# emstoudenmire/TNML

Measured on AMD Instinct MI355X. Metric: two-site bond updates/sec, higher is better.
Workload: dtype f64; 1 GPU; fixedL N=784, maxm=120, 60000 images (BASELINE config 3: its 60 000 images on 1 GPU instead of 8), Npass=4, lambda=0.001, minm=120, fp64 throughout; random-init W at m=maxm; timed bonds 405..202 (consecutive interior bonds, Label-carrying shiftE on each, m=119); global_images=60000, sites=784, maxm=120, parallelism=dp1 (image sharding + RCCL all-reduce), rccl_ranks=1

## Files before the change

### tnml_amd/csrc/kernels_grad.hip

```cpp
#include "tnml_internal.h"

typedef double f64x4g __attribute__((ext_vector_type(4)));

#define GQ_TI 32
#ifndef GQ_SLOT
#define GQ_SLOT(rgp) (2 * (rgp))
#endif
#ifndef GQ_PRIO
#define GQ_PRIO 3
#endif
#define GQ_RS 34
#define GQ_Q 32
#define GQ_E_D_N(NR) (32 * (NR) * GQ_RS)
#define GQ_Z_D (GQ_Q * GQ_RS)
#define GQ_W_D (4 * GQ_RS)
#define GQ_LDS_DOUBLES_N(NR) (2 * (GQ_E_D_N(NR) + GQ_Z_D + GQ_W_D))
#define GQ_LDS_DOUBLES GQ_LDS_DOUBLES_N(4)

struct GradQuadArgs {
    const double* EI; const double* phiI; const double* phiO;
    const double* EL; size_t EL_lstride;
    const double* dP;
    int NTp;
    int mI, mO, Kp, Np;
    double* slab;
    int ngroups, per, nchunks;
    long long* dbg = nullptr;
};

static __device__ __forceinline__ void gq_barrier() {
    asm volatile("s_waitcnt lgkmcnt(0)" ::: "memory");
    __builtin_amdgcn_s_barrier();
    asm volatile("" ::: "memory");
}

template <int ABL, int NR = 4>
__global__ __launch_bounds__(1024) void k_grad_quad(GradQuadArgs A) {
    static_assert(NR == 4 || NR == 2, "quad form or pair form");
    constexpr int GQ_E_D = GQ_E_D_N(NR);
    extern __shared__ __attribute__((aligned(16))) double gq_lds[];
    double* const Es = gq_lds;
    double* const Zs = Es + 2 * GQ_E_D;
    double* const Ws = Zs + 2 * GQ_Z_D;
    const int tid = threadIdx.x, lane = tid & 63, w = __builtin_amdgcn_readfirstlane(tid >> 6);
    const int b = blockIdx.x;
    const long long ts0 = (ABL == 5 || ABL == 6) ? (long long)wall_clock64() : 0;
    const int h = (b >> 3) & (NR - 1), grp = (b & 7) + 8 * (NR == 4 ? b >> 5 : b >> 4);
    if (grp >= A.ngroups) return;
    const int NTp = A.NTp;
    const int c0 = grp * A.per;
    const int nch = min(A.per, A.nchunks - c0);
    auto n_of = [&](int k) { return (size_t)(c0 + (k < nch ? k : nch - 1)) * GQ_TI; };

    const int rho = lane >> 4, x2 = 2 * (lane & 15);
    double2 pc[3];
    const unsigned pvoff = (unsigned)(((size_t)rho * NTp + x2) * sizeof(double));
    auto ld16 = [&](const double* ubase, unsigned voff) { return *reinterpret_cast<const double2*>(reinterpret_cast<const char*>(ubase) + voff); };
    const bool v0 = 4 * w + rho < A.mI, v1 = NR == 4 && 64 + 4 * w + rho < A.mI;
    const double* fO = A.phiO - 2 * (size_t)NTp;
    const double* fb = A.phiI < fO ? A.phiI : fO;
    const unsigned fvoff = pvoff + (unsigned)(((rho < 2 ? A.phiI : fO) - fb) * (ptrdiff_t)sizeof(double));
    auto piece_load = [&](size_t nE, double2 (&pc)[3]) {
        unsigned vo = pvoff, vf = fvoff;
        asm volatile("" : "+v"(vo), "+v"(vf));
        pc[0] = v0 ? ld16(A.EI + (size_t)(4 * w) * NTp + nE, vo) : make_double2(0., 0.);
        if (NR == 4) pc[1] = v1 ? ld16(A.EI + (size_t)(4 * (w + 16)) * NTp + nE, vo) : make_double2(0., 0.);
        if (w == 15) pc[2] = ld16(fb + nE, vf);
    };
    const int dst0 = (4 * w + rho) * GQ_RS + x2;
    auto piece_store = [&](int bufE, const double2 (&pc)[3]) {
        *reinterpret_cast<double2*>(Es + bufE * GQ_E_D + dst0) = pc[0];
        if (NR == 4) *reinterpret_cast<double2*>(Es + bufE * GQ_E_D + dst0 + 64 * GQ_RS) = pc[1];
        if (w == 15) {
            const int lI = 16 * (rho >> 1) + (lane & 15), lO = 16 * (2 + (rho & 1)) + (lane & 15);
            const double ix = __shfl(pc[2].x, lI), iy = __shfl(pc[2].y, lI), ox = __shfl(pc[2].x, lO), oy = __shfl(pc[2].y, lO);
            *reinterpret_cast<double2*>(Ws + bufE * GQ_W_D + rho * GQ_RS + x2) = make_double2(ix * ox, iy * oy);
        }
    };
    const int img = lane & 31, qs = lane >> 5;
    double el[2][5], dpv[5];
    const unsigned elvoff = (unsigned)(((size_t)(5 * qs) * A.EL_lstride + img) * sizeof(double));
    const unsigned dpvoff = (unsigned)(((size_t)(5 * qs) * NTp + img) * sizeof(double));
    const bool uv[2] = {GQ_Q * h + w < A.mO, GQ_Q * h + w + 16 < A.mO};
    auto el_load = [&](size_t n0, double (&el)[2][5], double (&dpv)[5]) {
        unsigned elvo = elvoff, dpvo = dpvoff;
        asm volatile("" : "+v"(elvo), "+v"(dpvo));
#pragma unroll
        for (int l = 0; l < 5; ++l) dpv[l] = *reinterpret_cast<const double*>(reinterpret_cast<const char*>(A.dP + (size_t)l * NTp + n0) + dpvo);
#pragma unroll
        for (int j = 0; j < 2; ++j) {
            const double* ub = A.EL + (size_t)(GQ_Q * h + w + 16 * j) * NTp + n0;
#pragma unroll
            for (int l = 0; l < 5; ++l)
                el[j][l] = !uv[j] ? 0. : (ABL == 1 ? 1.0 : *reinterpret_cast<const double*>(reinterpret_cast<const char*>(ub + (size_t)l * A.EL_lstride) + elvo));
        }
    };
    auto z_build = [&](int bufZ, const double (&el)[2][5], const double (&dpv)[5]) {
#pragma unroll
        for (int j = 0; j < 2; ++j) {
            double z = 0.;
#pragma unroll
            for (int l = 0; l < 5; ++l) z = fma(el[j][l], dpv[l], z);
            const double zo = __shfl_xor(z, 32);
            if (qs == 0) Zs[bufZ * GQ_Z_D + (w + 16 * j) * GQ_RS + img] = z + zo;
        }
    };

    const int rgp = w >> 2, J = w & 3;
    const int li = lane & 15, g = lane >> 4;
    const int sI = rgp >> 1, a0 = 16 * NR * (rgp & 1);
    const int eoff = (a0 + li) * GQ_RS + g;
    const int cc = 16 * J + li;
    const int zoff = (cc >> 1) * GQ_RS + g;
    const int woff = (2 * sI + (cc & 1)) * GQ_RS + g;
    {
        double2 pc0[3]; double el0[2][5], dpv0[5];
        piece_load(n_of(0), pc0);
        el_load(n_of(0), el0, dpv0);
        if (ABL != 6) { piece_load(n_of(1), pc); el_load(n_of(1), el, dpv); }
        piece_store(0, pc0);
        z_build(0, el0, dpv0);
        if (ABL == 6) { piece_load(n_of(1), pc); el_load(n_of(1), el, dpv); }
    }
    gq_barrier();
    const long long ts1 = (ABL == 5 || ABL == 6) ? (long long)wall_clock64() : 0;

    f64x4g acc[NR];
#pragma unroll
    for (int r = 0; r < NR; ++r) acc[r] = f64x4g{0., 0., 0., 0.};
    double en[NR], zn, on;
    auto frag_load = [&](int buf, int ks) {
        const double* Eb = Es + buf * GQ_E_D + eoff + 4 * ks;
#pragma unroll
        for (int r = 0; r < NR; ++r) en[r] = Eb[16 * r * GQ_RS];
        zn = Zs[buf * GQ_Z_D + zoff + 4 * ks];
        on = Ws[buf * GQ_W_D + woff + 4 * ks];
    };
    frag_load(0, 0);
    for (int k = 0; k < nch; ++k) {
        const int cur = k & 1, nxt = cur ^ 1;
#pragma unroll
        for (int ks = 0; ks < 8; ++ks) {
            if (ABL != 3 && ks == GQ_SLOT(rgp)) {
                __builtin_amdgcn_s_setprio(GQ_PRIO);
                piece_store(nxt, pc);
                z_build(nxt, el, dpv);
                piece_load(n_of(k + 2), pc);
                el_load(n_of(k + 2), el, dpv);
                __builtin_amdgcn_s_setprio(0);
                __builtin_amdgcn_sched_barrier(0);
            }
            double ec[NR];
#pragma unroll
            for (int r = 0; r < NR; ++r) ec[r] = en[r];
            const double bc = zn * on;
            __builtin_amdgcn_sched_barrier(0);
            if (ks < 7) frag_load(cur, ks + 1);
            __builtin_amdgcn_sched_barrier(0);
#pragma unroll
            for (int r = 0; r < NR; ++r) acc[r] = __builtin_amdgcn_mfma_f64_16x16x4f64(ec[r], bc, acc[r], 0, 0, 0);
            __builtin_amdgcn_sched_barrier(0);
        }
        gq_barrier();
        frag_load(nxt, 0);
    }

    const long long ts2 = (ABL == 5 || ABL == 6) ? (long long)wall_clock64() : 0;
    double* out = A.slab + (size_t)grp * A.Kp * A.Np;
    const int col = 2 * GQ_Q * h + cc;
    if (col < A.Np) {
#pragma unroll
        for (int r = 0; r < NR; ++r)
#pragma unroll
            for (int e4 = 0; e4 < 4; ++e4) {
                const int row = 2 * (a0 + 16 * r + g + 4 * e4) + sI;
                if (row < A.Kp) out[(size_t)row * A.Np + col] = acc[r][e4];
            }
    }
    if ((ABL == 5 || ABL == 6) && A.dbg) {
        asm volatile("s_waitcnt vmcnt(0)" ::: "memory");
        __syncthreads();
        if (tid == 0) { long long* d = A.dbg + 4 * (size_t)b; d[0] = ts0; d[1] = ts1; d[2] = ts2; d[3] = (long long)wall_clock64(); }
    }
}

static inline bool gq_pair_form(const Bgemm64Args& a) { return a.mI <= 64 && a.mO <= 64 && a.Kp <= 128 && a.Np <= 128; }

bool grad_quad_applies(const tnml_ctx* c, const Bgemm64Args& a) {
    if (!c->grad_quad || !a.EL || !a.env64 || a.L != 1 || a.w) return false;
    if (a.mI < 1 || a.mO < 1 || a.mI > 128 || a.mO > 128 || a.Kp < 2 * a.mI || a.Np < 2 * a.mO || a.Kp > 256 || a.Np > 256 || a.NTp % GQ_TI) return false;
    if (c->grad_quad == 1) {
        if (gq_pair_form(a)) {
            const int mm = a.mI * a.mO;
            if (!c->grad_pair || a.NTp < 15360 || mm < 33 * 33 || mm > 56 * 56) return false;
        } else if (a.NTp < 4096 || a.mI * a.mO < 72 * 72) return false;
    }
    if ((size_t)TNML_NL * a.EL_lstride * sizeof(double) >= ((size_t)1 << 32)) return false;
    return c->slab_bytes >= (size_t)64 * a.Kp * a.Np * sizeof(double);
}

template <int NR>
static int grad_quad_go(tnml_ctx* c, const GradQuadArgs& K, int grid) {
    const size_t lds = sizeof(double) * GQ_LDS_DOUBLES_N(NR);
    bool& done = NR == 4 ? c->attr_gq : c->attr_gp;
    if (!done) {
        if (hipFuncSetAttribute(reinterpret_cast<const void*>(k_grad_quad<0, NR>), hipFuncAttributeMaxDynamicSharedMemorySize, (int)lds) != hipSuccess)
            return tnml_fail(c, "grad_quad: cannot reserve %zu bytes of LDS", lds);
        done = true;
    }
    ProfScope ps(c, KC_GRAD_QUAD);
    hipLaunchKernelGGL((k_grad_quad<0, NR>), dim3(grid), dim3(1024), lds, c->stream, K);
    return 0;
}

int launch_grad_quad(tnml_ctx* c, const Bgemm64Args& a, double* G) {
    if (!c->cu_count) { hipDeviceProp_t pr; c->cu_count = hipGetDeviceProperties(&pr, c->cfg.device) == hipSuccess ? pr.multiProcessorCount : 256; }
    const bool pair = gq_pair_form(a) && c->grad_pair != 0;
    const int nwg = pair ? 2 : 4;
    GradQuadArgs K;
    K.EI = static_cast<const double*>(a.EI); K.phiI = static_cast<const double*>(a.phiI); K.phiO = static_cast<const double*>(a.phiO);
    K.EL = static_cast<const double*>(a.EL); K.EL_lstride = a.EL_lstride; K.dP = a.dPz; K.NTp = a.NTp;
    K.mI = a.mI; K.mO = a.mO; K.Kp = a.Kp; K.Np = a.Np;
    K.slab = static_cast<double*>(c->slab);
    K.nchunks = a.NTp / GQ_TI;
    int groups = c->cu_count / nwg;
    const int cap = (int)(c->slab_bytes / ((size_t)a.Kp * a.Np * sizeof(double)));
    if (groups > cap) groups = cap;
    if (c->bgemm_wgs > 0 && c->bgemm_wgs / nwg < groups) groups = c->bgemm_wgs / nwg > 0 ? c->bgemm_wgs / nwg : 1;
    if (groups > K.nchunks) groups = K.nchunks;
    K.per = (K.nchunks + groups - 1) / groups;
    K.ngroups = (K.nchunks + K.per - 1) / K.per;
    const int grid = 8 * nwg * ((K.ngroups + 7) / 8);
    if (pair) TCK(grad_quad_go<2>(c, K, grid));
    else      TCK(grad_quad_go<4>(c, K, grid));
    const size_t n = (size_t)a.Kp * a.Np;
    if (c->defer_slab) c->slab_pending = K.ngroups;
    else {
        ProfScope ps(c, KC_SLABRED);
        launch_slab_reduce64(c, static_cast<const double*>(c->slab), G, n, K.ngroups);
    }
    HIPCK(c, hipGetLastError());
    return 0;
}
```

### tnml_amd/csrc/tnml_core.hip

```cpp
#include <algorithm>
#include <climits>
#include <cmath>
#include <cstdarg>
#include <cstdlib>
#include <cstring>

#include "tnml_host.h"

static std::string g_create_err;

int tnml_fail(tnml_ctx* c, const char* fmt, ...) {
    char buf[512];
    va_list ap; va_start(ap, fmt); vsnprintf(buf, sizeof buf, fmt, ap); va_end(ap);
    if (c) { c->err = buf; if (c->local && c->coll_depth > 0) local_comm_abort(c); } else g_create_err = buf;
    return 1;
}
const char* tnml_last_error(const tnml_ctx* c) { return c ? c->err.c_str() : g_create_err.c_str(); }
const char* tnml_last_warning(const tnml_ctx* c) { return c ? c->warn.c_str() : ""; }

static hipEvent_t prof_event(tnml_ctx* c) {
    if (!c->prof_free.empty()) { hipEvent_t e = c->prof_free.back(); c->prof_free.pop_back(); return e; }
    hipEvent_t e; (void)hipEventCreate(&e); return e;
}
void prof_begin(tnml_ctx* c, int, hipEvent_t* e0, hipStream_t st) { *e0 = prof_event(c); (void)hipEventRecord(*e0, st ? st : c->stream); }
void prof_end(tnml_ctx* c, int kc, hipEvent_t e0, hipStream_t st) {
    hipEvent_t e1 = prof_event(c); (void)hipEventRecord(e1, st ? st : c->stream);
    c->prof_pending.push_back({e0, e1, kc});
    if (c->prof_pending.size() > 8192) prof_resolve(c);
}
void prof_resolve(tnml_ctx* c) {
    if (c->prof_pending.empty()) return;
    (void)hipStreamSynchronize(c->stream);
    for (auto& p : c->prof_pending) {
        float ms = 0.f;
        if (hipEventElapsedTime(&ms, p.e0, p.e1) == hipSuccess) { c->prof_ms[p.kc] += ms; c->prof_launches[p.kc] += 1; }
        c->prof_free.push_back(p.e0); c->prof_free.push_back(p.e1);
    }
    c->prof_pending.clear();
}
int tnml_profile_enable(tnml_ctx* c, int on) { prof_resolve(c); c->prof = on != 0; return 0; }
int tnml_profile_select(tnml_ctx* c, const char* class_name) {
    prof_resolve(c);
    if (!class_name || !*class_name) { c->prof_mask = 0xffffffffu; return 0; }
    unsigned mask = 0;
    const char* s = class_name;
    while (*s) {
        const char* e = strchr(s, ',');
        const size_t len = e ? (size_t)(e - s) : strlen(s);
        bool found = false;
        for (int i = 0; i < KC_COUNT; ++i) if (strlen(kclass_names[i]) == len && !strncmp(s, kclass_names[i], len)) { mask |= 1u << i; found = true; }
        if (!found) return tnml_fail(c, "tnml_profile_select: unknown kernel class in %s", class_name);
        s = e ? e + 1 : s + len;
    }
    c->prof_mask = mask;
    return 0;
}
int tnml_profile_count(tnml_ctx*) { return KC_COUNT; }
int tnml_profile_get(tnml_ctx* c, int idx, char* name64, int64_t* launches, double* total_ms) {
    if (idx < 0 || idx >= KC_COUNT) return tnml_fail(c, "profile index out of range");
    prof_resolve(c);
    if (name64) { strncpy(name64, kclass_names[idx], 63); name64[63] = 0; }
    if (launches) *launches = c->prof_launches[idx];
    if (total_ms) *total_ms = c->prof_ms[idx];
    return 0;
}
int tnml_profile_reset(tnml_ctx* c) {
    prof_resolve(c);
    for (int i = 0; i < KC_COUNT; ++i) { c->prof_launches[i] = 0; c->prof_ms[i] = 0.; }
    return 0;
}
enum OptKind { OPT_BOOL, OPT_INT, OPT_REAL };
enum OptHook { HK_NONE, HK_REUSE_P, HK_DEFER_TAIL, HK_CHECK_REPLICAS, HK_ENV_BUDGET, HK_COMM_TIMEOUT, HK_FAIL_SPLIT, HK_MISPREDICT, HK_SVD_PRINT, HK_CG_METHOD, HK_NOISE, HK_PREDICT_TILE };
struct OptDef {
    const char* name; const char* env; OptKind kind;
    int tnml_ctx::* ifield; double tnml_ctx::* rfield;
    double lo, hi; OptHook hook;
};
static const OptDef k_options[] = {
    {"fast_cg",          "TNML_FAST_CG",        OPT_BOOL, &tnml_ctx::fast_cg,             nullptr,          0, 1,       HK_NONE},
    {"reuse_p",          "TNML_REUSE_P",        OPT_BOOL, &tnml_ctx::reuse_p,             nullptr,          0, 1,       HK_REUSE_P},
    {"fuse_z",           "TNML_FUSE_Z",         OPT_BOOL, &tnml_ctx::fuse_z,              nullptr,          0, 1,       HK_NONE},
    {"merged_cg",        "TNML_MERGED_CG",      OPT_INT,  &tnml_ctx::merged_cg,           nullptr,          0, 2,       HK_NONE},
    {"defer_tail",       "TNML_DEFER_TAIL",     OPT_BOOL, &tnml_ctx::defer_tail,          nullptr,          0, 1,       HK_DEFER_TAIL},
    {"check_replicas",   "TNML_CHECK_REPLICAS", OPT_INT,  &tnml_ctx::check_replicas_mode, nullptr,          0, 2,       HK_CHECK_REPLICAS},
    {"fused_fwd",        "TNML_FUSED_FWD",      OPT_INT,  &tnml_ctx::fused_fwd,           nullptr,          0, INT_MAX, HK_NONE},
    {"fwd_res",          "TNML_FWD_RES",        OPT_INT,  &tnml_ctx::fwd_res,             nullptr,          0, 3,       HK_NONE},
    {"shift_res",        "TNML_SHIFT_RES",      OPT_INT,  &tnml_ctx::shift_res,           nullptr,          0, 2,       HK_NONE},
    {"shift_skip",       "TNML_SHIFT_SKIP",     OPT_BOOL, &tnml_ctx::shift_skip,          nullptr,          0, 1,       HK_NONE},
    {"res_grid",         nullptr,               OPT_INT,  &tnml_ctx::res_grid,            nullptr,          0, INT_MAX, HK_NONE},
    {"res_pace",         "TNML_RES_PACE",       OPT_INT,  &tnml_ctx::res_pace,            nullptr,          0, 4,       HK_NONE},
    {"grad_quad",        "TNML_GRAD_QUAD",      OPT_INT,  &tnml_ctx::grad_quad,           nullptr,          0, 2,       HK_NONE},
    {"grad_pair",        "TNML_GRAD_PAIR",      OPT_BOOL, &tnml_ctx::grad_pair,           nullptr,          0, 1,       HK_NONE},
    {"bgemm_wgs",        "TNML_BGEMM_WGS",      OPT_INT,  &tnml_ctx::bgemm_wgs,           nullptr,          0, INT_MAX, HK_NONE},
    {"bgemm_per",        "TNML_BGEMM_PER",      OPT_INT,  &tnml_ctx::bgemm_per,           nullptr,          0, 1 << 20, HK_NONE},
    {"sytrd_exit",       nullptr,               OPT_BOOL, &tnml_ctx::sytrd_exit,          nullptr,          0, 1,       HK_NONE},
    {"bgs_chol",         "TNML_BGS_CHOL",       OPT_BOOL, &tnml_ctx::bgs_chol,            nullptr,          0, 1,       HK_NONE},
    {"spec_split",       "TNML_SPEC_SPLIT",     OPT_BOOL, &tnml_ctx::spec_split,          nullptr,          0, 1,       HK_NONE},
    {"debug_fail_split", nullptr,               OPT_INT,  &tnml_ctx::debug_fail_split,    nullptr,         -1, INT_MAX, HK_FAIL_SPLIT},
    {"spec_predict",     "TNML_SPEC_PREDICT",   OPT_BOOL, &tnml_ctx::spec_predict,        nullptr,          0, 1,       HK_NONE},
    {"debug_mispredict", nullptr,               OPT_INT,  &tnml_ctx::debug_mispredict,    nullptr,         -1, INT_MAX, HK_MISPREDICT},
    {"bf16_grad",        nullptr,               OPT_BOOL, &tnml_ctx::bf16_grad,           nullptr,          0, 1,       HK_NONE},
    {"bf16_once",        nullptr,               OPT_BOOL, &tnml_ctx::bf16_once,           nullptr,          0, 1,       HK_NONE},
    {"env_async",        nullptr,               OPT_BOOL, &tnml_ctx::env_async,           nullptr,          0, 1,       HK_NONE},
    {"env_budget_mb",    nullptr,               OPT_INT,  nullptr,                        nullptr,          0, INT_MAX, HK_ENV_BUDGET},
    {"comm_timeout_s",   nullptr,               OPT_INT,  &tnml_ctx::comm_timeout_s,      nullptr,          1, INT_MAX, HK_COMM_TIMEOUT},
    {"cg_method",        nullptr,               OPT_INT,  &tnml_ctx::cg_method,           nullptr,          0, 2,       HK_CG_METHOD},
    {"debug_nudge_rank", nullptr,               OPT_INT,  &tnml_ctx::debug_nudge_rank,    nullptr,         -1, INT_MAX, HK_NONE},
    {"mc_spin_max",      nullptr,               OPT_INT,  &tnml_ctx::mc_spin_max,         nullptr,         -1, INT_MAX, HK_NONE},
    {"svd_print",        "TNML_SVD_PRINT",      OPT_INT,  &tnml_ctx::svd_print,           nullptr,         -2, INT_MAX, HK_SVD_PRINT},
    {"predict_chunk",    nullptr,               OPT_INT,  &tnml_ctx::predict_chunk,       nullptr,          1, 1 << 20, HK_NONE},
    {"predict_tile",     nullptr,               OPT_INT,  &tnml_ctx::predict_tile,        nullptr,          0, 64,      HK_PREDICT_TILE},
    {"predict_dtype",    nullptr,               OPT_INT,  &tnml_ctx::predict_dtype,       nullptr,          0, 1,       HK_NONE},
    {"response_chunk",   nullptr,               OPT_INT,  &tnml_ctx::response_chunk,      nullptr,          1, 1 << 20, HK_NONE},
    {"gradient_chunk",   nullptr,               OPT_INT,  &tnml_ctx::gradient_chunk,      nullptr,          1, 1 << 20, HK_NONE},
    {"fg64_cfg",         "TNML_FG64_CFG",       OPT_INT,  &tnml_ctx::opt_fg64_cfg,        nullptr,          0, 2,       HK_NONE},
    {"ldot_cfg",         "TNML_LDOT_CFG",       OPT_INT,  &tnml_ctx::opt_ldot_cfg,        nullptr,          0, 2,       HK_NONE},
    {"pcut",             nullptr,               OPT_REAL, nullptr,                        &tnml_ctx::pcut,  0, HUGE_VAL, HK_NONE},
    {"noise",            nullptr,               OPT_REAL, nullptr,                        &tnml_ctx::noise, 0, HUGE_VAL, HK_NOISE},
};
static int apply_option(tnml_ctx* c, const OptDef& d, double v, const char* who, const char* what) {
    if (d.kind != OPT_BOOL && !(v >= d.lo && v <= d.hi)) {
        if (d.hi >= INT_MAX) return tnml_fail(c, "%s: %s = %.15g, must be >= %.15g", who, what, v, d.lo);
        return tnml_fail(c, "%s: %s = %.15g, must be in %.15g..%.15g", who, what, v, d.lo, d.hi);
    }
    switch (d.hook) {
        case HK_NONE: break;
        case HK_REUSE_P: c->p_valid = false; break;
        case HK_DEFER_TAIL: if (c->pend_count) return tnml_fail(c, "defer_tail: a bond update is in flight"); break;
        case HK_CHECK_REPLICAS: c->check_replicas = v != 0; break;
        case HK_ENV_BUDGET: c->env_budget_bytes = (long)v << 20; break;
        case HK_COMM_TIMEOUT: local_comm_set_timeout(c, (int)v); break;
        case HK_FAIL_SPLIT: c->spec_splits = 0; break;
        case HK_MISPREDICT: c->pred_splits = 0; break;
        case HK_SVD_PRINT: c->svd_calls = 0; break;
        case HK_CG_METHOD:
            if (v >= 1 && !c->single()) return tnml_fail(c, "cg_method: 0 (conj) or, in TNML_MODE_SINGLE, 1 (fast_conj) / 2 (exact)");
            break;
        case HK_PREDICT_TILE:
            if (v != 0 && v != 16 && v != 32 && v != 64) return tnml_fail(c, "%s: %s = %.15g, must be 0, 16, 32 or 64", who, what, v);
            break;
        case HK_NOISE:
            if (v >= 1e-14 && !c->single()) return tnml_fail(c, "noise: the density-matrix split exists in the per-label variant only (single.h:648-672)");
            if (v >= 1e-14 && !c->env64()) return tnml_fail(c, "noise: needs fp64 environments (dtype f64)");
            break;
    }
    if (d.ifield) c->*d.ifield = d.kind == OPT_BOOL ? v != 0 : (int)v;
    if (d.rfield) c->*d.rfield = v;
    return 0;
}
static int set_option(tnml_ctx* c, const char* who, const char* name, double v, bool real) {
    if (!c || !name) return tnml_fail(c, "%s: null argument", who);
    for (const OptDef& d : k_options)
        if ((d.kind == OPT_REAL) == real && !strcmp(d.name, name)) return apply_option(c, d, v, who, name);
    return tnml_fail(c, "%s: unknown option %s", who, name);
}
int tnml_set_option(tnml_ctx* c, const char* name, int value) { return set_option(c, "tnml_set_option", name, value, false); }
int tnml_set_option_real(tnml_ctx* c, const char* name, double value) { return set_option(c, "tnml_set_option_real", name, value, true); }
int tnml_synchronize(tnml_ctx* c) { HIPCK(c, hipStreamSynchronize(c->stream)); if (c->copy_stream) HIPCK(c, hipStreamSynchronize(c->copy_stream)); return ipc_comm_check(c); }
int64_t tnml_device_bytes(tnml_ctx* c) { return c->bytes; }
int64_t tnml_replica_repairs(tnml_ctx* c) { return c->replica_repairs; }
static void resolve_redo_events(std::vector<std::pair<hipEvent_t, hipEvent_t>>& ev, double* sum_ms) {
    for (size_t k = 0; k < ev.size();) {
        float ms = 0.f;
        if (hipEventElapsedTime(&ms, ev[k].first, ev[k].second) == hipSuccess) {
            *sum_ms += ms;
            (void)hipEventDestroy(ev[k].first); (void)hipEventDestroy(ev[k].second);
            ev.erase(ev.begin() + k);
        } else { (void)hipGetLastError(); ++k; }
    }
}
int tnml_spec_predict_stats(tnml_ctx* c, int64_t* predicted, int64_t* mispredicted, double* redo_ms) {
    if (!c) return tnml_fail(c, "tnml_spec_predict_stats: null argument");
    resolve_redo_events(c->pred_redo_events, &c->pred_redo_ms);
    if (predicted) *predicted = c->pred_splits_total;
    if (mispredicted) *mispredicted = c->mispredicted;
    if (redo_ms) *redo_ms = c->pred_redo_ms;
    return 0;
}
int tnml_truncate_device(tnml_ctx* c, const double* evals_ascending, int n, int maxm, int minm, double cutoff, int m_pred, int* m, int* wrong) {
    if (!c || !evals_ascending || !m || !wrong) return tnml_fail(c, "tnml_truncate_device: null argument");
    if (n < 1 || n > (1 << 20)) return tnml_fail(c, "tnml_truncate_device: n = %d, must be in 1..%d", n, 1 << 20);
    if (c->pend_count > 0) return tnml_fail(c, "tnml_truncate_device: a bond update is in flight (tnml_bond_update_end first)");
    HIPCK(c, hipSetDevice(c->cfg.device));
    double* d = nullptr;
    HIPCK(c, hipMalloc((void**)&d, sizeof(double) * ((size_t)n + 3)));
    double out[3] = {-1., -1., -1.};
    int rc = 0;
    if (hipMemcpyAsync(d, evals_ascending, sizeof(double) * n, hipMemcpyHostToDevice, c->stream) != hipSuccess) rc = tnml_fail(c, "tnml_truncate_device: copy to the device failed");
    if (!rc) rc = launch_truncate_verdict(c, d, n, maxm, minm, cutoff, m_pred, d + n, d + n + 2);
    if (!rc && hipMemcpyAsync(out, d + n, sizeof out, hipMemcpyDeviceToHost, c->stream) != hipSuccess) rc = tnml_fail(c, "tnml_truncate_device: copy from the device failed");
    if (!rc && hipStreamSynchronize(c->stream) != hipSuccess) rc = tnml_fail(c, "tnml_truncate_device: the kernel failed");
    (void)hipFree(d);
    if (rc) return rc;
    if (out[1] != out[2]) return tnml_fail(c, "tnml_truncate_device: the mirrored verdict %g differs from the carried word %g", out[1], out[2]);
    *m = (int)out[0]; *wrong = out[1] != 0. ? 1 : 0;
    return 0;
}
int tnml_split_stats(tnml_ctx* c, int64_t* spec_splits, int64_t* roll_backs, double* roll_back_ms) {
    resolve_redo_events(c->redo_events, &c->redo_ms);
    resolve_redo_events(c->pred_redo_events, &c->pred_redo_ms);
    if (spec_splits) *spec_splits = c->spec_splits_total;
    if (roll_backs) *roll_backs = c->spec_redos;
    if (roll_back_ms) *roll_back_ms = c->redo_ms + c->pred_redo_ms;
    return 0;
}
int tnml_svd_stats(tnml_ctx* c, int64_t* fallbacks, int64_t* cluster_repairs, double* d0, double* d1) {
    if (fallbacks) *fallbacks = c->svd_fallbacks;
    if (cluster_repairs) *cluster_repairs = c->svd_cholqr;
    if (d0) *d0 = c->svd_last_dev0;
    if (d1) *d1 = c->svd_last_dev1;
    return 0;
}

int tnml_truncate(const double* P, int origm, int maxm, int minm, double cutoff, double* truncerr) {
    if (origm <= 1) { if (truncerr) *truncerr = 0.; return origm; }
    int n = origm - 1;
    double te = 0.;
    while (n >= maxm) { te += P[n]; --n; }
    double scale = 0.;
    for (int j = 0; j < origm; ++j) scale += P[j];
    if (scale == 0.) scale = 1.;
    while (n >= 0 && te + P[n] < cutoff * scale && n >= minm) { te += P[n]; --n; }
    if (n < 0) n = 0;
    if (truncerr) *truncerr = te / scale;
    return n + 1;
}
void tnml_sweepnext(int* b, int* ha, int N) {
    const int inc = (*ha == 1) ? +1 : -1;
    *b += inc;
    if (*b == ((*ha == 1) ? N : 0)) { *b -= inc; ++*ha; }
}
void tnml_shard_bounds(int64_t NT_total, int nranks, int rank, int64_t* begin, int64_t* end) {
    const int64_t th = NT_total / nranks;
    *begin = th * rank;
    *end = (rank == nranks - 1) ? NT_total : th * (rank + 1);
}

static void ctx_plan(tnml_ctx* c, const tnml_config& cfg) {
    c->cfg = cfg;
    c->N = cfg.N; c->NT = cfg.NT_local; c->maxm = cfg.maxm;
    c->c0 = cfg.mode == TNML_MODE_SINGLE ? -1 : cfg.N / 2;
    c->NTp = (cfg.NT_local + TNML_NTPAD - 1) / TNML_NTPAD * TNML_NTPAD;
    const size_t NTp = c->NTp, m = c->maxm;
    const int Kmax = c->bf16() ? (2 * c->maxm + 31) / 32 * 32 : ru16(2 * c->maxm);
    c->mcap = (size_t)TNML_NL * Kmax * Kmax;
// ... 184 lines not shown
```

### tnml_amd/csrc/tnml_internal.h

```cpp
#pragma once
#include <hip/hip_runtime.h>
#include <rocblas/rocblas.h>
#include <rocsolver/rocsolver.h>
#include <rccl/rccl.h>

#include <algorithm>
#include <cstdint>
#include <cstdio>
#include <string>
#include <utility>
#include <vector>

#include "../../include/tnml.h"

#define TNML_NTPAD 256

enum KClass {
    KC_FGEMM_FWD = 0, KC_FGEMM_SHIFT, KC_LABELDOT, KC_ZPRIME, KC_BGEMM, KC_SLABRED, KC_PACK, KC_VEC,
    KC_SMALLGEMM, KC_SVD, KC_ALLREDUCE, KC_PUPDATE, KC_FWD_FUSED, KC_FWD_RES, KC_GRAD_QUAD, KC_CHAIN, KC_EVAL_TALLY, KC_SITE_RESP, KC_SITE_BWD, KC_SITE_GRAD, KC_STEP_NORM, KC_SITE_STEP, KC_COUNT
};
static const char* const kclass_names[KC_COUNT] = {
    "fgemm_fwd", "fgemm_shift", "labeldot", "zprime", "bgemm", "slab_reduce", "pack", "cg_vec",
    "small_gemm", "svd", "allreduce", "p_update", "fwd_fused", "fwd_res", "grad_quad", "chain", "eval_tally", "site_resp", "site_bwd", "site_grad", "step_norm", "site_step"};

// ... 32 lines not shown
#define TNML_CARRY 16
#define TNML_FPSLOT 32
#define TNML_CARRYN 24
#define TNML_SPECSLOT 28
#define TNML_PREDSLOT 29

struct BondPlan {
    int b = -1;
    int kind = 0;
    int mL = 0, mR = 0;
    int mI = 0, mO = 0;
    int Kp = 0, Np = 0, LB = 1;
    const void* EI = nullptr; const void* phiI = nullptr;
    const void* EX = nullptr; const void* phiO = nullptr;
    size_t msize() const { return (size_t)LB * Kp * Np; }
};

struct ProfPending { hipEvent_t e0, e1; int kc; };
struct SiteUndo { int j = 0; double* old = nullptr; int ml = 0, mr = 0; };
struct PendingReport {
    tnml_bond_report rep; double lambda_cost = 0.; hipEvent_t ev = nullptr, ev2 = nullptr; bool fp = false;
    int b = 0, ha = 0; tnml_sweep_params sp{};
    bool spec = false; int split_n = 0, split_mk = 0; int nundo = 0; SiteUndo undo[2];
    bool p_saved = false;
    bool pred = false; int m_pred = 0;
    int dn_pairs = 0, cost_rows = 0; bool trace_mirrored = false, carry_direct = false;
    bool ho = false; hipEvent_t ev_ho = nullptr; SiteT ho_site[2];
};
struct HeldOut {
    struct tnml_ctx* train = nullptr;
    hipEvent_t ev_copied = nullptr;
    bool copy_recorded = false;
    hipEvent_t ev_done[2] = {nullptr, nullptr};
    double* host = nullptr;
    int slot = 0;
    int bond[2] = {0, 0}, half[2] = {0, 0};
};

template <typename E> struct ChainSite;

struct StreamWs {
    int cap = 0; int64_t bytes = 0;
    ChainSite<double>* tab = nullptr;
    double* w = nullptr; int* pred = nullptr;
    uint8_t *raw8 = nullptr, *x8 = nullptr;
    double *rawphi = nullptr, *xphi = nullptr;
    uint8_t* mraw = nullptr;
    uint16_t* codes = nullptr; double* mtab = nullptr;
};

struct tnml_ctx {
    tnml_config cfg;
    int N = 0, NT = 0, NTp = 0, c0 = 0, maxm = 0;
    hipStream_t stream = nullptr;
    int fused_fwd = 1;
    int cg_method = 0;
    double pcut = 1e-8;
    double noise = 0.;
    double* noise_ws = nullptr;
    int sytrd_exit = 1;
    rocblas_handle blas = nullptr;
    ncclComm_t comm = nullptr;
    struct LocalComm* local = nullptr;
    struct IpcComm* ipc = nullptr;
    bool multi() const { return comm != nullptr || local != nullptr || ipc != nullptr; }
    std::string err;
    std::string warn;
    int64_t bytes = 0;

    void* phi = nullptr;
    int* label = nullptr;
    void* ones = nullptr;
    bool data_set = false;

    std::vector<SiteT> W;
    std::vector<EnvSlot> env;
    std::vector<EnvSlab> slabs;
    size_t small_elems = 0, big_elems = 0;

    void* U = nullptr;
    void* P = nullptr;
    void* dP = nullptr;
    void* Pp = nullptr;
    int fuse_z = 1;
    int fast_cg = 1;
    int reuse_p = 1; bool p_valid = false;
    long env_budget_bytes = 0;
    int env_protect[4] = {0, 0, 0, 0};
    long env_spills = 0, env_fetches = 0, env_prefetches = 0;
    hipStream_t copy_stream = nullptr;
    hipEvent_t ev_compute = nullptr;
    int env_async = 1;
    int bf16_once = 1;
    unsigned short* ebt = nullptr; unsigned short* mbt = nullptr; size_t ebt_cap = 0, mbt_cap = 0;
    const void* ebt_src = nullptr; int ebt_m = 0; unsigned long ebt_epoch = 0, env_epoch = 1;
    bool attr_bf16e = false;
    int bf16_grad = 1;
    int bgs_chol = 1;
    int coll_depth = 0;
    int comm_timeout_s = 120;
    int opt_fg64_cfg = 0, opt_ldot_cfg = 0;
    void* Zp = nullptr;
    float* Mf = nullptr;
    void* slab = nullptr;
    size_t slab_bytes = 0;
    bool f64() const { return cfg.dtype == TNML_F64 || cfg.dtype == TNML_F64_E32; }
    int bf16() const { return cfg.dtype == TNML_BF16 ? 1 : (cfg.dtype == TNML_BF16X3 ? 2 : 0); }
    bool env64() const { return cfg.dtype == TNML_F64; }
    bool single() const { return cfg.mode == TNML_MODE_SINGLE; }
    int nl() const { return single() ? 1 : TNML_NL; }
    int target() const { return single() ? cfg.target_label : -1; }
    size_t esz() const { return f64() ? 8 : 4; }
    size_t eesz() const { return env64() ? 8 : 4; }
    double* partials = nullptr;
    double* partials2 = nullptr;
    bool defer_slab = false;
    int slab_pending = 0;
    bool rr_from_part = false;
    int partial_cap = 0;
    int part_n = 0;
    double *vB = nullptr, *vR = nullptr, *vP = nullptr;
    double* arbuf = nullptr;
    double* tail = nullptr;
    double* vG = nullptr;
    double* locals = nullptr;
    int merged_cg = 1;
    int defer_tail = 1;
    int carry_slot = -1;
    long allreduce_calls = 0, bcast_calls = 0;
    double* scal = nullptr;
    double* cgtrace = nullptr;
    double* vpart = nullptr;
    int cg_pass = 0;
    int rr_slot = 0;
    double* h_scal = nullptr;
    double *tB = nullptr, *tB2 = nullptr;
    size_t mcap = 0;
    size_t sM_cap = 0;
    double *sM = nullptr, *sG = nullptr, *sD = nullptr, *sE = nullptr, *sF = nullptr;
    double *sE2 = nullptr, *sTau = nullptr, *sV = nullptr, *sC = nullptr;
    double *sW = nullptr, *sScr = nullptr, *sS = nullptr, *sCm = nullptr, *sQ1 = nullptr, *sDev = nullptr;
    void* mc_xbuf = nullptr;
    unsigned mc_epoch = 0;
    int mc_spin_max = -1;
    bool attr_sr[32] = {false}, attr_fr[4][32] = {{false}};
    int res_pace = 0;
    int fwd_res = 1;
    int shift_res = 1;
    int shift_skip = 1;
    uint8_t* zs_ord = nullptr; uint8_t* zs_nz = nullptr; int* zs_cnt = nullptr;
    std::vector<int> zs_groups;
    int res_grid = 0;
    int grad_quad = 1;
    bool attr_gq = false, attr_gp = false;
    int grad_pair = 1;
    int bgemm_per = 0;
    int bgemm_wgs = 0;
    unsigned* counters = nullptr;
    double* Ppart = nullptr;
    bool attr_sytrd = false, attr_invit = false, attr_fused = false;
    int cu_count = 0;
    int spec_split = 1; bool force_safe = false; long spec_redos = 0, spec_splits = 0;
    int debug_fail_split = -1;
    long spec_splits_total = 0; double redo_ms = 0.; std::vector<std::pair<hipEvent_t, hipEvent_t>> redo_events;
    int spec_predict = 0;
    int debug_mispredict = -1;
    long pred_splits = 0, pred_splits_total = 0, mispredicted = 0; double pred_redo_ms = 0.;
    std::vector<std::pair<hipEvent_t, hipEvent_t>> pred_redo_events;
    struct BondHist { int n[2] = {0, 0}, m[2] = {0, 0}; };
    std::vector<BondHist> bond_hist;
    double* psave = nullptr;
    std::vector<double*> spare_small, spare_big;
    double* hrep = nullptr;
    double* hmir = nullptr;
    double* hcost = nullptr;
    int last_dn_pairs = 0;
    size_t hrep_stride = 0;
    double svd_last_dev0 = 0., svd_last_dev1 = 0.;
    long svd_fallbacks = 0, svd_cholqr = 0;
    int svd_print = -2, svd_calls = 0, svd_dumped = 0;
    std::string svd_dump;
    double last_bnorm = 0.;
    int* sInfo = nullptr;
    unsigned long long* fprint = nullptr;
    int check_replicas_mode = 1;
    long replica_repairs = 0;
    int debug_nudge_rank = -1;
    bool check_replicas = true;
    int svd_n = 0;

    BondPlan plan;
    int currb = -1;
    PendingReport pend[2];
    int pend_tail = 0, pend_count = 0;
    bool tail_zeroed = false;
    tnml_ctx* ho = nullptr;
    HeldOut* held = nullptr;
    bool sweep_start = false;

    int predict_chunk = TNML_PREDICT_CHUNK_DEFAULT;
    int predict_tile = 0;
    bool attr_chain[2][2] = {};
    int predict_dtype = 0;
    float* pk_w32 = nullptr; size_t pk_w32_cap = 0;
    ChainSite<float>* pk_tab32 = nullptr;
    int* pk_flag = nullptr;
    float* pk_xphi32 = nullptr;
    int64_t pk_mtab32_bytes = 0;
    float* pk_mtab32 = nullptr;
    StreamWs pk;
    double* pk_park = nullptr; size_t pk_park_elems = 0;
    int* pk_lab = nullptr;
    EvalAcc* pk_acc = nullptr;
    int64_t pk_map_bytes = 0;
    int response_chunk = TNML_RESPONSE_CHUNK_DEFAULT;
    bool attr_response[2] = {};
    StreamWs rs;
    int* rs_which = nullptr;
    int* rs_rowoff = nullptr;
    double *rs_out = nullptr, *rs_outT = nullptr;
    double* rs_tape = nullptr; size_t rs_tape_rows = 0;
    int gradient_chunk = TNML_GRADIENT_CHUNK_DEFAULT;
    bool attr_sitegrad[2] = {};
    StreamWs sg;
    int* sg_lab = nullptr; double* sg_coef = nullptr;
    int* sg_rowoff = nullptr;
    long long* sg_goff = nullptr; int* sg_blk0 = nullptr;
    double* sg_grad = nullptr; size_t sg_grad_elems = 0;
    double *sg_tape = nullptr, *sg_tape2 = nullptr; size_t sg_tape_rows = 0;
    int st_method = -1;
    std::vector<int> st_shape;
    size_t st_elems = 0; int st_nblk = 0, st_nwg = 0;
    double *st_m = nullptr, *st_v = nullptr;
    double* st_bsum = nullptr;
    double* st_res = nullptr;
    int* st_wg0 = nullptr;
    EvalAcc* st_acc = nullptr;
    int64_t st_t = 0; double st_p1 = 1., st_p2 = 1.;
    int64_t st_bytes = 0;
    bool im_set = false;
    tnml_input_map im = {};
    std::vector<double> im_table;

    bool prof = false;
    unsigned prof_mask = 0xffffffffu;
    int64_t prof_launches[KC_COUNT] = {0};
    double prof_ms[KC_COUNT] = {0};
    std::vector<ProfPending> prof_pending;
    std::vector<hipEvent_t> prof_free;
};

int tnml_fail(tnml_ctx* c, const char* fmt, ...);
void prof_begin(tnml_ctx* c, int kc, hipEvent_t* e0, hipStream_t st = nullptr);
void prof_end(tnml_ctx* c, int kc, hipEvent_t e0, hipStream_t st = nullptr);
void prof_resolve(tnml_ctx* c);

#define HIPCK(c, expr) do { hipError_t e_ = (expr); if (e_ != hipSuccess) return tnml_fail((c), "%s failed: %s (%s:%d)", #expr, hipGetErrorString(e_), __FILE__, __LINE__); } while (0)
#define TCK(expr) do { int r_ = (expr); if (r_) return r_; } while (0)
#define SYNCK(c, st) do { HIPCK((c), hipStreamSynchronize(st)); TCK(ipc_comm_check(c)); } while (0)

struct ProfScope {
    tnml_ctx* c; int kc; hipEvent_t e0 = nullptr; hipStream_t st;
    bool on;
    ProfScope(tnml_ctx* c_, int kc_, hipStream_t st_ = nullptr) : c(c_), kc(kc_), st(st_), on(c_->prof && ((c_->prof_mask >> kc_) & 1u)) { if (on) prof_begin(c, kc, &e0, st); }
    ~ProfScope() { if (on) prof_end(c, kc, e0, st); }
};

struct FgemmArgs {
    const float* EI; size_t EI_lstride; int mI;
    const float* phiI;
    const float* M; size_t M_lstride; int Kp, Np;
    const float* phiO;
    float* out; size_t out_lstride; int mO;
    int NTp; int L;
};
int launch_fgemm(tnml_ctx* c, const FgemmArgs& a);
size_t bf16e_env_elems(int maxm, int NTp, int split);
size_t bf16e_m_elems(int maxm, int split);
int launch_fgemm_bf16e(tnml_ctx* c, const float* EI, int mI, const float* phiI, const double* vec, int Kp, int Np, const float* phiO, float* out, int mO);

struct BgemmArgs {
    const float* EI; int mI; const float* phiI;
    const float* Zq; int mO; const float* phiO;
    const float* w; size_t w_lstride;
    int Kp, Np, NTp, L;
    int bf16 = 0;
};
int launch_bgemm(tnml_ctx* c, const BgemmArgs& a, double* G);

struct Fgemm64Args {
    const void* EI; size_t EI_lstride; int mI;
    const void* phiI;
    const double* M; size_t M_lstride; int Kp, Np;
    const void* phiO;
    double* out; size_t out_lstride; int mO;
    int NTp; int L;
    int env64;
    int out32 = 0;
    int n_off = 0, n_cnt = 0;
    hipStream_t st = nullptr;
    int kclass = -1;
};
int launch_fgemm64(tnml_ctx* c, const Fgemm64Args& a);
struct Bgemm64Args {
    const void* EI; int mI; const void* phiI;
    const double* Zq64; const void* Zq32; int mO; const void* phiO;
    const void* EL; size_t EL_lstride; const double* dPz;
// ... 303 lines not shown
```

Before: 404.7 bond updates/s.

## Add prefetching grad_quad kernel with LDS DMA triple buffering and register ring

Adds k_grad_quad_pf, a variant of the gradient quad/pair kernel that stages E and auxiliary data into LDS with global_load_lds_dwordx4 across three buffers and keeps EL values in a register ring loaded one chunk ahead. The intent is to hide global-load latency behind the MFMA loop using explicit vmcnt waits and a raised priority for the shared-data stage. By default it is used only for the pair form (NR==2), selected through a new grad_prefetch option. The cost is more LDS per block, fragile hand-written inline asm, and 32-bit offset limits that are checked before the kernel is chosen.

```diff
diff --git a/tnml_amd/csrc/kernels_grad.hip b/tnml_amd/csrc/kernels_grad.hip
--- a/tnml_amd/csrc/kernels_grad.hip
+++ b/tnml_amd/csrc/kernels_grad.hip
@@ -1,6 +1,7 @@
 #include "tnml_internal.h"
 
 typedef double f64x4g __attribute__((ext_vector_type(4)));
+typedef double f64x2g __attribute__((ext_vector_type(2)));
 
 #define GQ_TI 32
 #ifndef GQ_SLOT
@@ -184,6 +185,195 @@
     }
 }
 
+#define GP_PAIR_B 2304
+#define GP_E_B(NR) (4 * (NR) * GP_PAIR_B)
+#define GP_AUX_B 4096
+#define GP_RL 5
+#define GP_LDS_BYTES(NR) (3 * GP_E_B(NR) + 3 * GP_AUX_B + 2 * (GQ_Z_D + GQ_W_D) * (int)sizeof(double))
+
+template <int N> static __device__ __forceinline__ void gp_vmcnt() { asm volatile("s_waitcnt vmcnt(%0)" :: "n"(N) : "memory"); }
+
+template <int NR>
+__global__ __launch_bounds__(1024) void k_grad_quad_pf(GradQuadArgs A) {
+    static_assert(NR == 4 || NR == 2, "quad form or pair form");
+    constexpr int NP = NR / 2;
+    constexpr int EB = GP_E_B(NR);
+    extern __shared__ __attribute__((aligned(16))) double gq_lds[];
+    char* const lds = reinterpret_cast<char*>(gq_lds);
+    const unsigned lds0 = __builtin_amdgcn_readfirstlane((unsigned)(size_t)((__attribute__((address_space(3))) char*)gq_lds));
+    char* const Xs = lds + 3 * EB;
+    double* const Zs = reinterpret_cast<double*>(Xs + 3 * GP_AUX_B);
+    double* const Ws = Zs + 2 * GQ_Z_D;
+    const int tid = threadIdx.x, lane = tid & 63, w = __builtin_amdgcn_readfirstlane(tid >> 6);
+    const int b = blockIdx.x;
+    const int h = (b >> 3) & (NR - 1), grp = (b & 7) + 8 * (NR == 4 ? b >> 5 : b >> 4);
+    if (grp >= A.ngroups) return;
+    const int NTp = A.NTp;
+    const int c0 = grp * A.per;
+    const int nch = min(A.per, A.nchunks - c0);
+    auto n_of = [&](int k) { return (size_t)(c0 + (k < nch ? k : nch - 1)) * GQ_TI; };
+
+    auto dma16 = [&](const double* base, unsigned voff, unsigned dst) {
+        unsigned keep;
+        asm volatile("s_mov_b32 %0, m0\n\ts_mov_b32 m0, %2\n\ts_nop 0\n\tglobal_load_lds_dwordx4 %1, %3\n\ts_mov_b32 m0, %0" : "=&s"(keep) : "v"(voff), "s"(dst), "s"(base) : "memory");
+    };
+    auto ev_off = [&](int ln, int i) {
+        const int q = NP * w + i;
+        const int row = min(16 * (q >> 2) + 8 * (q & 1) + (ln & 7), A.mI - 1);
+        return ((unsigned)row * (unsigned)NTp + (unsigned)(16 * ((q >> 1) & 1) + 2 * (ln >> 3))) * (unsigned)sizeof(double);
+    };
+    auto e_dst = [&](int i) { const int q = NP * w + i; return (unsigned)((q >> 1) * GP_PAIR_B + (q & 1) * 1152); };
+    const bool xw = w < 4;
+    const double* fO = A.phiO - 2 * (size_t)NTp;
+    const double* fb = A.phiI < fO ? A.phiI : fO;
+    const double* const abase = w == 0 ? fb : A.dP;
+    auto av_off = [&](int ln) {
+        const int rho = ln >> 4, x2 = 2 * (ln & 15);
+        if (w == 0) return (unsigned)((((size_t)rho * NTp + x2) + (size_t)((rho < 2 ? A.phiI : fO) - fb)) * sizeof(double));
+        return ((unsigned)min(4 * w - 4 + rho, TNML_NL - 1) * (unsigned)NTp + (unsigned)x2) * (unsigned)sizeof(double);
+    };
+    auto pieces = [&](int ln, int kE, int bufE, int kX, int bufX) {
+        if (xw) dma16(abase + n_of(kX), av_off(ln), lds0 + (unsigned)(3 * EB + bufX * GP_AUX_B + w * 1024));
+#pragma unroll
+        for (int i = 0; i < NP; ++i) dma16(A.EI + n_of(kE), ev_off(ln, i), lds0 + (unsigned)(bufE * EB) + e_dst(i));
+    };
+    const bool uv[2] = {GQ_Q * h + w < A.mO, GQ_Q * h + w + 16 < A.mO};
+    const unsigned eloff[2] = {uv[0] ? (unsigned)(GQ_Q * h + w) * (unsigned)NTp : 0u, uv[1] ? (unsigned)(GQ_Q * h + w + 16) * (unsigned)NTp : 0u};
+    auto ring_load = [&](int ln, size_t n0, f64x2g (&e)[GP_RL]) {
+        const int lg = ln >> 4;
+        const unsigned elvoff = ((unsigned)(5 * (lg & 1)) * (unsigned)A.EL_lstride + (lg >> 1 ? eloff[1] : eloff[0]) + (unsigned)(2 * (ln & 15))) * (unsigned)sizeof(double);
+#pragma unroll
+        for (int i = 0; i < GP_RL; ++i) {
+#if defined(GP_PROBE) && GP_PROBE == 2
+            const double* bp = A.EL + (size_t)i * A.EL_lstride;
+#else
+            const double* bp = A.EL + (size_t)i * A.EL_lstride + n0;
+#endif
+            asm volatile("global_load_dwordx4 %0, %1, %2" : "=v"(e[i]) : "v"(elvoff), "s"(bp) : "memory");
+        }
+    };
+    auto ring_wait = [&](auto nn, auto nx, f64x2g (&e)[GP_RL]) {
+        constexpr int N = decltype(nn)::value, NX = decltype(nx)::value;
+        if (NX != N && xw) gp_vmcnt<NX>(); else gp_vmcnt<N>();
+        asm volatile("" : "+v"(e[0]), "+v"(e[1]), "+v"(e[2]), "+v"(e[3]), "+v"(e[4]) :: "memory");
+    };
+    auto share = [&](auto nn, auto nx, int bufZ, int bufXr, int kE, int bufE, int kX, int bufX, f64x2g (&e)[GP_RL]) {
+        int ln = lane;
+        asm volatile("" : "+v"(ln));
+        const double* xr = reinterpret_cast<const double*>(Xs + bufXr * GP_AUX_B);
+        if (w == 15) {
+            const int rho = ln >> 4, x2 = 2 * (ln & 15);
+            const double2 fi = *reinterpret_cast<const double2*>(xr + (rho >> 1) * GQ_TI + x2), fo = *reinterpret_cast<const double2*>(xr + (2 + (rho & 1)) * GQ_TI + x2);
+            *reinterpret_cast<double2*>(Ws + bufZ * GQ_W_D + rho * GQ_RS + x2) = make_double2(fi.x * fo.x, fi.y * fo.y);
+        }
+        ring_wait(nn, nx, e);
+        const int p2 = 2 * (ln & 15), lg = ln >> 4;
+        const double* dp = xr + (4 + 5 * (lg & 1)) * GQ_TI + p2;
+        double2 z = make_double2(0., 0.);
+#pragma unroll
+        for (int i = 0; i < GP_RL; ++i) { const double2 d = *reinterpret_cast<const double2*>(dp + i * GQ_TI); z.x = fma(e[i].x, d.x, z.x); z.y = fma(e[i].y, d.y, z.y); }
+        const double zox = __shfl_xor(z.x, 16), zoy = __shfl_xor(z.y, 16);
+        if (!(lg & 1)) {
+            const bool ok = lg >> 1 ? uv[1] : uv[0];
+            *reinterpret_cast<double2*>(Zs + bufZ * GQ_Z_D + (w + 16 * (lg >> 1)) * GQ_RS + p2) = ok ? make_double2(z.x + zox, z.y + zoy) : make_double2(0., 0.);
+        }
+        pieces(ln, kE, bufE, kX, bufX);
+        ring_load(ln, n_of(kX), e);
+    };
+
+    const int rgp = w >> 2, J = w & 3;
+    const int li = lane & 15, g = lane >> 4;
+    const int sI = rgp >> 1, a0 = 16 * NR * (rgp & 1);
+    const int cc = 16 * J + li;
+    const int zoff = (cc >> 1) * GQ_RS + g;
+    const int woff = (2 * sI + (cc & 1)) * GQ_RS + g;
+    int eaddr = 2 * NR * (rgp & 1) * GP_PAIR_B + (li >> 3) * 1152 + (g >> 1) * 128 + (li & 7) * 16 + (g & 1) * 8;
+
+    f64x2g elA[GP_RL], elB[GP_RL];
+    {
+        int ln = lane;
+        asm volatile("" : "+v"(ln));
+        if (xw) {
+            dma16(abase + n_of(0), av_off(ln), lds0 + (unsigned)(3 * EB + 0 * GP_AUX_B + w * 1024));
+            dma16(abase + n_of(1), av_off(ln), lds0 + (unsigned)(3 * EB + 1 * GP_AUX_B + w * 1024));
+        }
+#pragma unroll
+        for (int i = 0; i < NP; ++i) dma16(A.EI + n_of(0), ev_off(ln, i), lds0 + e_dst(i));
+        ring_load(ln, n_of(0), elA);
+        ring_load(ln, n_of(1), elB);
+    }
+    gp_vmcnt<2 * GP_RL>();
+    gq_barrier();
+    using icrl = std::integral_constant<int, GP_RL>;
+    share(icrl(), icrl(), 0, 0, 1, 1, 2, 2, elA);
+    gq_barrier();
+
+    f64x4g acc[NR];
+#pragma unroll
+    for (int r = 0; r < NR; ++r) acc[r] = f64x4g{0., 0., 0., 0.};
+    double en[NR], zn, on;
+    auto frag_load = [&](int buf, int ks) {
+        const char* Eb = lds + eaddr + (ks >> 2) * GP_PAIR_B + (ks & 3) * 256;
+#pragma unroll
+        for (int r = 0; r < NR; ++r) en[r] = *reinterpret_cast<const double*>(Eb + 2 * r * GP_PAIR_B);
+        zn = Zs[buf * GQ_Z_D + zoff + 4 * ks];
+        on = Ws[buf * GQ_W_D + woff + 4 * ks];
+    };
+    auto stage = [&](auto curc, int k, int i3, f64x2g (&e)[GP_RL]) {
+        constexpr int cur = decltype(curc)::value, nxt = cur ^ 1;
+        const int i3n = i3 == 2 ? 0 : i3 + 1, i3p = i3 == 0 ? 2 : i3 - 1;
+#pragma unroll
+        for (int ks = 0; ks < 8; ++ks) {
+            if (ks == GQ_SLOT(rgp)) {
+                __builtin_amdgcn_s_setprio(GQ_PRIO);
+                share(std::integral_constant<int, NP + GP_RL>(), std::integral_constant<int, 1 + NP + GP_RL>(), nxt, i3n, k + 2, i3p, k + 3, i3, e);
+                __builtin_amdgcn_s_setprio(0);
+                __builtin_amdgcn_sched_barrier(0);
+            }
+            double ec[NR];
+#pragma unroll
+            for (int r = 0; r < NR; ++r) ec[r] = en[r];
+            const double bc = zn * on;
+            __builtin_amdgcn_sched_barrier(0);
+            if (ks < 7) frag_load(cur, ks + 1);
+            __builtin_amdgcn_sched_barrier(0);
+#pragma unroll
+            for (int r = 0; r < NR; ++r) acc[r] = __builtin_amdgcn_mfma_f64_16x16x4f64(ec[r], bc, acc[r], 0, 0, 0);
+            __builtin_amdgcn_sched_barrier(0);
+        }
+        if (xw) gp_vmcnt<GP_RL + 1 + NP + GP_RL>(); else gp_vmcnt<GP_RL + NP + GP_RL>();
+        gq_barrier();
+        eaddr += i3 == 2 ? -2 * EB : EB;
+        frag_load(nxt, 0);
+    };
+    frag_load(0, 0);
+    {
+        const std::integral_constant<int, 0> even; const std::integral_constant<int, 1> odd;
+        int k = 0, i3 = 0;
+        for (; k + 1 < nch; k += 2) {
+            stage(even, k, i3, elB);
+            i3 = i3 == 2 ? 0 : i3 + 1;
+            stage(odd, k + 1, i3, elA);
+            i3 = i3 == 2 ? 0 : i3 + 1;
+        }
+        if (k < nch) stage(even, k, i3, elB);
+    }
+    asm volatile("s_waitcnt vmcnt(0)" :: "v"(elA[0]), "v"(elA[1]), "v"(elA[2]), "v"(elA[3]), "v"(elA[4]), "v"(elB[0]), "v"(elB[1]), "v"(elB[2]), "v"(elB[3]), "v"(elB[4]) : "memory");
+    __builtin_amdgcn_sched_barrier(0);
+
+    double* out = A.slab + (size_t)grp * A.Kp * A.Np;
+    const int col = 2 * GQ_Q * h + cc;
+    if (col < A.Np) {
+#pragma unroll
+        for (int r = 0; r < NR; ++r)
+#pragma unroll
+            for (int e4 = 0; e4 < 4; ++e4) {
+                const int a = a0 + 16 * r + g + 4 * e4, row = 2 * a + sI;
+                if (row < A.Kp) out[(size_t)row * A.Np + col] = a < A.mI ? acc[r][e4] : 0.;
+            }
+    }
+}
+
 static inline bool gq_pair_form(const Bgemm64Args& a) { return a.mI <= 64 && a.mO <= 64 && a.Kp <= 128 && a.Np <= 128; }
 
 bool grad_quad_applies(const tnml_ctx* c, const Bgemm64Args& a) {
@@ -201,15 +391,19 @@
 
 template <int NR>
 static int grad_quad_go(tnml_ctx* c, const GradQuadArgs& K, int grid) {
-    const size_t lds = sizeof(double) * GQ_LDS_DOUBLES_N(NR);
-    bool& done = NR == 4 ? c->attr_gq : c->attr_gp;
+    const bool pf = (c->grad_prefetch == 2 || (c->grad_prefetch == 0 && NR == 2)) && (size_t)K.mI * K.NTp * sizeof(double) < ((size_t)1 << 32)
+                    && (size_t)(TNML_NL + 1) * K.EL_lstride * sizeof(double) < ((size_t)1 << 32) && (size_t)K.mO * K.NTp <= K.EL_lstride;
+    const size_t lds = pf ? (size_t)GP_LDS_BYTES(NR) : sizeof(double) * GQ_LDS_DOUBLES_N(NR);
+    const void* fn = pf ? reinterpret_cast<const void*>(k_grad_quad_pf<NR>) : reinterpret_cast<const void*>(k_grad_quad<0, NR>);
+    bool& done = pf ? (NR == 4 ? c->attr_gq_pf : c->attr_gp_pf) : (NR == 4 ? c->attr_gq : c->attr_gp);
     if (!done) {
-        if (hipFuncSetAttribute(reinterpret_cast<const void*>(k_grad_quad<0, NR>), hipFuncAttributeMaxDynamicSharedMemorySize, (int)lds) != hipSuccess)
+        if (hipFuncSetAttribute(fn, hipFuncAttributeMaxDynamicSharedMemorySize, (int)lds) != hipSuccess)
             return tnml_fail(c, "grad_quad: cannot reserve %zu bytes of LDS", lds);
         done = true;
     }
     ProfScope ps(c, KC_GRAD_QUAD);
-    hipLaunchKernelGGL((k_grad_quad<0, NR>), dim3(grid), dim3(1024), lds, c->stream, K);
+    if (pf) hipLaunchKernelGGL((k_grad_quad_pf<NR>), dim3(grid), dim3(1024), lds, c->stream, K);
+    else    hipLaunchKernelGGL((k_grad_quad<0, NR>), dim3(grid), dim3(1024), lds, c->stream, K);
     return 0;
 }
 
diff --git a/tnml_amd/csrc/tnml_core.hip b/tnml_amd/csrc/tnml_core.hip
--- a/tnml_amd/csrc/tnml_core.hip
+++ b/tnml_amd/csrc/tnml_core.hip
@@ -91,6 +91,7 @@
     {"res_pace",         "TNML_RES_PACE",       OPT_INT,  &tnml_ctx::res_pace,            nullptr,          0, 4,       HK_NONE},
     {"grad_quad",        "TNML_GRAD_QUAD",      OPT_INT,  &tnml_ctx::grad_quad,           nullptr,          0, 2,       HK_NONE},
     {"grad_pair",        "TNML_GRAD_PAIR",      OPT_BOOL, &tnml_ctx::grad_pair,           nullptr,          0, 1,       HK_NONE},
+    {"grad_prefetch",    "TNML_GRAD_PREFETCH",  OPT_INT,  &tnml_ctx::grad_prefetch,       nullptr,          0, 2,       HK_NONE},
     {"bgemm_wgs",        "TNML_BGEMM_WGS",      OPT_INT,  &tnml_ctx::bgemm_wgs,           nullptr,          0, INT_MAX, HK_NONE},
     {"bgemm_per",        "TNML_BGEMM_PER",      OPT_INT,  &tnml_ctx::bgemm_per,           nullptr,          0, 1 << 20, HK_NONE},
     {"sytrd_exit",       nullptr,               OPT_BOOL, &tnml_ctx::sytrd_exit,          nullptr,          0, 1,       HK_NONE},
diff --git a/tnml_amd/csrc/tnml_internal.h b/tnml_amd/csrc/tnml_internal.h
--- a/tnml_amd/csrc/tnml_internal.h
+++ b/tnml_amd/csrc/tnml_internal.h
@@ -208,7 +208,8 @@
     std::vector<int> zs_groups;
     int res_grid = 0;
     int grad_quad = 1;
-    bool attr_gq = false, attr_gp = false;
+    bool attr_gq = false, attr_gp = false, attr_gq_pf = false, attr_gp_pf = false;
+    int grad_prefetch = 0;
     int grad_pair = 1;
     int bgemm_per = 0;
     int bgemm_wgs = 0;
```

After: 399.8 bond updates/s. -1.2%, worse.
